# hliangzhao/torch-on-k8s

Hardware: AMD Instinct MI355X
Metric: tokens_per_s (higher is better)
Workload: dtype bf16; 1 GPU; model=llama3-8b, global_batch=8, seq_len=4096, parallelism=dp1, attn_impl=hip

## Files before the change

### torch_on_k8s_amd/models/llama.py

```python
from __future__ import annotations

import secrets
from dataclasses import dataclass, asdict

import torch
import torch.nn as nn
import torch.nn.functional as F

from torch_on_k8s_amd import ops


@dataclass
class LlamaConfig:
    name: str = "llama3-8b"
    vocab_size: int = 128256
    hidden_size: int = 4096
    intermediate_size: int = 14336
    num_layers: int = 32
    num_heads: int = 32
    num_kv_heads: int = 8
    head_dim: int = 128
    max_seq_len: int = 8192
    rope_theta: float = 500000.0
    rms_eps: float = 1e-5
    tie_embeddings: bool = False
    attn_impl: str = "hip"
    init_std: float = 0.02

    def to_dict(self):
        return asdict(self)


PRESETS = {
    "llama3-8b": LlamaConfig(),
    "llama-tiny": LlamaConfig(
        name="llama-tiny", vocab_size=512, hidden_size=256,
        intermediate_size=512, num_layers=2, num_heads=4, num_kv_heads=2,
        head_dim=64, max_seq_len=256, rope_theta=10000.0),
    "llama-1b": LlamaConfig(
        name="llama-1b", vocab_size=32000, hidden_size=2048,
        intermediate_size=5504, num_layers=16, num_heads=16, num_kv_heads=8,
        head_dim=128, max_seq_len=4096, rope_theta=500000.0),
}


def get_config(name: str, **overrides) -> LlamaConfig:
    cfg = PRESETS[name]
    if overrides:
        d = cfg.to_dict()
        d.update(overrides)
        cfg = LlamaConfig(**d)
    return cfg


class RMSNorm(nn.Module):
    def __init__(self, hidden: int, eps: float):
        super().__init__()
        self.weight = nn.Parameter(torch.ones(hidden))
        self.eps = eps

    def forward(self, x):
        return ops.rmsnorm(x, self.weight, self.eps)


def build_rope_table(cfg: LlamaConfig, seq_len: int, device) -> tuple[torch.Tensor, torch.Tensor]:
    half = cfg.head_dim // 2
    inv_freq = 1.0 / (cfg.rope_theta ** (torch.arange(0, half, dtype=torch.float64) / half))
    t = torch.arange(seq_len, dtype=torch.float64)
    ang = torch.outer(t, inv_freq)
    return (ang.cos().float().contiguous().to(device),
            ang.sin().float().contiguous().to(device))


class Attention(nn.Module):

    def __init__(self, cfg: LlamaConfig):
        super().__init__()
        self.cfg = cfg
        H, D = cfg.num_heads, cfg.head_dim
        Hkv = cfg.num_kv_heads
        self.qkv_proj = nn.Linear(cfg.hidden_size, (H + 2 * Hkv) * D,
                                  bias=False)
        self.o_proj = nn.Linear(H * D, cfg.hidden_size, bias=False)

    def project_qkv(self, x, cos, sin):
        cfg = self.cfg
        qkv = self.qkv_proj(x)
        return ops.qkv_rope(qkv, cos, sin, cfg.num_heads, cfg.num_kv_heads,
                            cfg.head_dim)

    def forward(self, x, cos, sin):
        B, S, _ = x.shape
        cfg = self.cfg
        q, k, v = self.project_qkv(x, cos, sin)
        if cfg.attn_impl == "sdpa" and x.is_cuda:
            rep = cfg.num_heads // cfg.num_kv_heads
            qt = q.transpose(1, 2)
            kt = k.transpose(1, 2).repeat_interleave(rep, dim=1)
            vt = v.transpose(1, 2).repeat_interleave(rep, dim=1)
            o = F.scaled_dot_product_attention(qt, kt, vt, is_causal=True)
            o = o.transpose(1, 2).contiguous()
        else:
            o = ops.attention(q, k, v, causal=True)
        return self.o_proj(o.reshape(B, S, cfg.num_heads * cfg.head_dim))


class MLP(nn.Module):

    def __init__(self, cfg: LlamaConfig):
        super().__init__()
        self.gate_up_proj = nn.Linear(cfg.hidden_size,
                                      2 * cfg.intermediate_size, bias=False)
        self.down_proj = nn.Linear(cfg.intermediate_size, cfg.hidden_size, bias=False)

    def forward(self, x):
        return self.down_proj(ops.swiglu(self.gate_up_proj(x)))


class Block(nn.Module):

    def __init__(self, cfg: LlamaConfig):
        super().__init__()
        self.input_norm = RMSNorm(cfg.hidden_size, cfg.rms_eps)
        self.attn = Attention(cfg)
        self.post_attn_norm = RMSNorm(cfg.hidden_size, cfg.rms_eps)
        self.mlp = MLP(cfg)

    def forward(self, x, res, cos, sin):
        h, xr = ops.rmsnorm_residual(x, res, self.input_norm.weight,
                                     self.input_norm.eps)
        a = self.attn(h, cos, sin)
        h2, xr2 = ops.rmsnorm_residual(a, xr, self.post_attn_norm.weight,
                                       self.post_attn_norm.eps)
        return self.mlp(h2), xr2


class LlamaModel(nn.Module):

    def __init__(self, cfg: LlamaConfig, activation_checkpointing: bool = False):
        super().__init__()
        self.cfg = cfg
        self.activation_checkpointing = activation_checkpointing
        self.embed_tokens = nn.Embedding(cfg.vocab_size, cfg.hidden_size)
        self.layers = nn.ModuleList(Block(cfg) for _ in range(cfg.num_layers))
        self.norm = RMSNorm(cfg.hidden_size, cfg.rms_eps)
        self.lm_head = nn.Linear(cfg.hidden_size, cfg.vocab_size, bias=False)
        if cfg.tie_embeddings:
            self.lm_head.weight = self.embed_tokens.weight
        self._rope_cache: tuple[int, torch.Tensor, torch.Tensor] | None = None
        self.reset_parameters()

    def reset_parameters(self):
        std = self.cfg.init_std
        for m in self.modules():
            if isinstance(m, nn.Linear):
                nn.init.normal_(m.weight, mean=0.0, std=std)
            elif isinstance(m, nn.Embedding):
                nn.init.normal_(m.weight, mean=0.0, std=std)
            elif isinstance(m, RMSNorm):
                nn.init.ones_(m.weight)
        scale = (2 * self.cfg.num_layers) ** -0.5
        for blk in self.layers:
            with torch.no_grad():
                blk.attn.o_proj.weight.mul_(scale)
                blk.mlp.down_proj.weight.mul_(scale)

    def _rope(self, S: int, device):
        if self._rope_cache is None or self._rope_cache[0] != S or \
                self._rope_cache[1].device != device:
            cos, sin = build_rope_table(self.cfg, S, device)
            self._rope_cache = (S, cos, sin)
        return self._rope_cache[1], self._rope_cache[2]

    def forward_hidden(self, input_ids: torch.Tensor) -> torch.Tensor:
        B, S = input_ids.shape
        cos, sin = self._rope(S, input_ids.device)
        x = self.embed_tokens(input_ids)
        res = None
        for blk in self.layers:
            if self.activation_checkpointing and self.training:
                x, res = torch.utils.checkpoint.checkpoint(
                    blk, x, res, cos, sin, use_reentrant=False)
            else:
                x, res = blk(x, res, cos, sin)
        y, _ = ops.rmsnorm_residual(x, res, self.norm.weight, self.norm.eps)
        return y

    def forward(self, input_ids: torch.Tensor,
                labels: torch.Tensor | None = None):
        x = self.forward_hidden(input_ids)
        logits = self.lm_head(x)
        if labels is None:
            return logits
        return ops.cross_entropy(logits, labels)

    @torch.no_grad()
    def generate(self, input_ids: torch.Tensor, max_new_tokens: int = 32,
                 temperature: float = 0.0,
                 use_graph: bool | None = None) -> torch.Tensor:
        cfg = self.cfg
        B, S0 = input_ids.shape
        dev = input_ids.device
        dtype = self.embed_tokens.weight.dtype
        Tmax = S0 + max_new_tokens
        Hkv, Hq, D = cfg.num_kv_heads, cfg.num_heads, cfg.head_dim
        kc = [torch.zeros(B, Tmax, Hkv, D, dtype=dtype, device=dev)
              for _ in self.layers]
        vc = [torch.zeros(B, Tmax, Hkv, D, dtype=dtype, device=dev)
              for _ in self.layers]
        cos, sin = build_rope_table(cfg, Tmax, dev)

        def run_block(blk, i, x, pos0, T):
            B_, s, _ = x.shape
            h = blk.input_norm(x)
            q, k, v = blk.attn.project_qkv(
                h, cos[pos0:pos0 + s].contiguous(),
                sin[pos0:pos0 + s].contiguous())
            kc[i][:, pos0:pos0 + s] = k
            vc[i][:, pos0:pos0 + s] = v
            if s > 1:
                o = ops.attention(q, k, v, causal=True)
            else:
                o = ops.attention_decode(q[:, 0], kc[i], vc[i], T)
                o = o.view(B_, 1, Hq, D)
            x = x + blk.attn.o_proj(o.reshape(B_, s, Hq * D))
            x = x + blk.mlp(blk.post_attn_norm(x))
            return x

        def next_token(logits):
            if temperature and temperature > 0:
                probs = torch.softmax(logits.float() / temperature, dim=-1)
                return torch.multinomial(probs, 1)
            return logits.argmax(-1, keepdim=True)

        x = self.embed_tokens(input_ids)
        for i, blk in enumerate(self.layers):
            x = run_block(blk, i, x, 0, S0)
        logits = self.lm_head(self.norm(x[:, -1:]))[:, -1]
        tokens = [next_token(logits)]

        if use_graph is None:
            use_graph = (dev.type == "cuda" and not temperature and
                         max_new_tokens >= 8)

        if not use_graph:
            for step in range(1, max_new_tokens):
                pos = S0 + step - 1
                x = self.embed_tokens(tokens[-1])
                for i, blk in enumerate(self.layers):
                    x = run_block(blk, i, x, pos, pos + 1)
                logits = self.lm_head(self.norm(x))[:, -1]
                tokens.append(next_token(logits))
            return torch.cat([input_ids] + tokens, dim=1)

        token_buf = tokens[0].clone()
        pos_long = torch.tensor([S0], dtype=torch.long, device=dev)
        t32 = torch.zeros((), dtype=torch.int32, device=dev)

        def decode_step():
            t32.copy_((pos_long[0] + 1).to(torch.int32))
            x = self.embed_tokens(token_buf)
            cs = torch.index_select(cos, 0, pos_long).contiguous()
            sn = torch.index_select(sin, 0, pos_long).contiguous()
            for i, blk in enumerate(self.layers):
                h = blk.input_norm(x)
                q, k, v = blk.attn.project_qkv(h, cs, sn)
                kc[i].index_copy_(1, pos_long, k)
                vc[i].index_copy_(1, pos_long, v)
                o = ops.attention_decode(q[:, 0], kc[i], vc[i], 0, T_dev=t32)
                x = x + blk.attn.o_proj(o.view(B, 1, Hq * D))
                x = x + blk.mlp(blk.post_attn_norm(x))
            logits = self.lm_head(self.norm(x))[:, -1]
            nxt = logits.argmax(-1, keepdim=True)
            token_buf.copy_(nxt)
# ... 164 lines not shown
```

### torch_on_k8s_amd/ops/__init__.py

```python
from __future__ import annotations

import torch

try:
    from . import _C
except ImportError:
    _C = None


def hip_ext_available() -> bool:
    return _C is not None


def _require_ext(op: str):
    if _C is None:
        raise RuntimeError(
            f"torch_on_k8s_amd HIP extension is required for {op} on GPU but "
            "is not built. Run: PYTORCH_ROCM_ARCH=gfx950 python setup.py "
            "build_ext --inplace"
        )
    return _C


def rmsnorm_ref(x: torch.Tensor, w: torch.Tensor, eps: float) -> torch.Tensor:
    xf = x.float()
    r = torch.rsqrt(xf.pow(2).mean(-1, keepdim=True) + eps)
    return (xf * r * w.float()).to(x.dtype)


class _RMSNormFn(torch.autograd.Function):
    @staticmethod
    def forward(ctx, x, w, eps):
        if x.is_cuda:
            y, invr = _require_ext("rmsnorm").rmsnorm_fwd(x, w, eps)
        else:
            xf = x.float()
            invr = torch.rsqrt(xf.pow(2).mean(-1) + eps).reshape(-1)
            y = (xf * invr.view(*x.shape[:-1], 1) * w.float()).to(x.dtype)
        ctx.save_for_backward(x, w, invr)
        return y

    @staticmethod
    def backward(ctx, dy):
        x, w, invr = ctx.saved_tensors
        dy = dy.contiguous()
        if x.is_cuda:
            dx, dw = _C.rmsnorm_bwd(x, w, dy, invr)
        else:
            xf, wf, dyf = x.float(), w.float(), dy.float()
            H = x.shape[-1]
            r = invr.view(*x.shape[:-1], 1)
            c = (dyf * wf * xf).sum(-1, keepdim=True)
            dx = (r * (wf * dyf - xf * (r * r / H) * c)).to(x.dtype)
            dw = (dyf * xf * r).reshape(-1, H).sum(0)
        return dx, dw.to(w.dtype), None


def rmsnorm(x: torch.Tensor, w: torch.Tensor, eps: float = 1e-5) -> torch.Tensor:
    return _RMSNormFn.apply(x.contiguous(), w, eps)


class _RMSNormResFn(torch.autograd.Function):

    @staticmethod
    def forward(ctx, x, res, w, eps):
        if x.is_cuda:
            y, xr, invr = _require_ext("rmsnorm_res").rmsnorm_res_fwd(
                x, res, w, eps)
        else:
            xr = x + res if res is not None else x
            xf = xr.float()
            invr = torch.rsqrt(xf.pow(2).mean(-1) + eps).reshape(-1)
            y = (xf * invr.view(*xr.shape[:-1], 1) * w.float()).to(x.dtype)
        ctx.save_for_backward(xr, w, invr)
        ctx.has_res = res is not None
        return y, xr

    @staticmethod
    def backward(ctx, dy, dxr):
        xr, w, invr = ctx.saved_tensors
        dy = dy.contiguous()
        if dxr is not None:
            dxr = dxr.contiguous()
# ... 392 lines not shown
        if logits.dtype != torch.bfloat16:
            raise TypeError(
                f"sample_tokens: GPU logits must be bfloat16, got "
                f"{logits.dtype}")
        return _require_ext("sample_tokens").sample_tokens(
            logits, temperature, top_k, top_p, seed, counter, u)
    B = logits.shape[0]
    out = torch.empty(B, dtype=torch.long)
    lf = logits.double()
    for b in range(B):
        ub = (float(u[b]) if u is not None
              else sample_uniform(int(seed[b]), int(counter[b])))
        out[b] = _sample_row_cpu(lf[b], float(temperature[b]), int(top_k[b]),
                                 float(top_p[b]), ub)
    return out


class _LayerNormFn(torch.autograd.Function):
    @staticmethod
    def forward(ctx, x, w, b, eps):
        if x.is_cuda:
            y, mu, rstd = _require_ext("layernorm").layernorm_fwd(x, w, b, eps)
        else:
            xf = x.float()
            mu = xf.mean(-1)
            var = xf.var(-1, unbiased=False)
            rstd = torch.rsqrt(var + eps)
            y = (((xf - mu.unsqueeze(-1)) * rstd.unsqueeze(-1)) * w.float() +
                 b.float()).to(x.dtype)
            mu, rstd = mu.reshape(-1), rstd.reshape(-1)
        ctx.save_for_backward(x, w, mu, rstd)
        return y

    @staticmethod
    def backward(ctx, dy):
        x, w, mu, rstd = ctx.saved_tensors
        dy = dy.contiguous()
        if x.is_cuda:
            dx, dw, db = _C.layernorm_bwd(x, w, dy, mu, rstd)
        else:
            H = x.shape[-1]
            xf, wf, dyf = x.float(), w.float(), dy.float()
            muv = mu.view(*x.shape[:-1], 1)
            rs = rstd.view(*x.shape[:-1], 1)
            xhat = (xf - muv) * rs
            dyw = dyf * wf
            a1 = dyw.mean(-1, keepdim=True)
            a2 = (dyw * xhat).mean(-1, keepdim=True)
            dx = (rs * (dyw - a1 - xhat * a2)).to(x.dtype)
            dw = (dyf * xhat).reshape(-1, H).sum(0)
            db = dyf.reshape(-1, H).sum(0)
        return dx, dw.to(w.dtype), db.to(w.dtype), None


def layernorm(x: torch.Tensor, w: torch.Tensor, b: torch.Tensor,
              eps: float = 1e-5) -> torch.Tensor:
    return _LayerNormFn.apply(x.contiguous(), w, b, eps)


class _FusedCEFn(torch.autograd.Function):
    @staticmethod
    def forward(ctx, logits, labels):
        loss, lse = _require_ext("cross_entropy").ce_fwd(logits, labels)
        ctx.save_for_backward(logits, labels, lse)
        return loss.mean()

    @staticmethod
    def backward(ctx, grad_out):
        logits, labels, lse = ctx.saved_tensors
        gscale = (grad_out.float() / logits.numel() * logits.size(-1)) \
            .reshape(())
        dlogits = _C.ce_bwd(logits, labels, lse, gscale.contiguous())
        return dlogits, None


def cross_entropy(logits: torch.Tensor, labels: torch.Tensor) -> torch.Tensor:
    if logits.is_cuda and logits.dtype == torch.bfloat16:
        return _FusedCEFn.apply(logits.contiguous().view(-1, logits.shape[-1]),
                                labels.reshape(-1).int())
    return torch.nn.functional.cross_entropy(
        logits.float().view(-1, logits.shape[-1]), labels.reshape(-1))


__all__ = [
    "rmsnorm", "rmsnorm_ref", "apply_rope", "rope_ref", "fused_adamw_",
    "attention", "attention_ref", "cross_entropy", "layernorm",
    "qkv_rope", "qkv_rope_ref", "swiglu", "swiglu_ref",
    "hip_ext_available",
    "grad_sumsq_blocks", "grad_sumsq_", "grad_norm_finalize_",
    "attention_decode_ragged", "qkv_rope_append_",
    "decode_ragged_splits", "decode_ragged_chunk",
    "sample_tokens", "sample_uniform", "philox4x32_10",
]
```

### torch_on_k8s_amd/ops/csrc/bindings.cpp

```cpp
#include <torch/extension.h>
#include <ATen/hip/impl/HIPStreamMasqueradingAsCUDA.h>
#include <hip/hip_runtime.h>

extern "C" {
hipError_t tok_rmsnorm_fwd(const void* x, const void* w, void* y, float* invr,
                           long nrows, int H, float eps, hipStream_t stream);
int tok_rmsnorm_dw_rsplit(long nrows, int H);
hipError_t tok_rmsnorm_bwd(const void* x, const void* w, const void* dy,
                           const float* invr, void* dx, float* dw_f32,
                           float* dw_ws, long nrows, int H,
                           hipStream_t stream);
hipError_t tok_rmsnorm_res_fwd(const void* x, const void* res, const void* w,
                               void* xr, void* y, float* invr, long nrows,
                               int H, float eps, hipStream_t stream);
hipError_t tok_rmsnorm_res_bwd(const void* xr, const void* w, const void* dy,
                               const void* dxr_in, const float* invr,
                               void* dx, float* dw_f32, float* dw_ws,
                               long nrows, int H, hipStream_t stream);
hipError_t tok_swiglu_fwd(const void* gu, void* out, long rows, int I,
                          hipStream_t stream);
hipError_t tok_swiglu_bwd(const void* dout, const void* gu, void* dgu,
                          long rows, int I, hipStream_t stream);
hipError_t tok_qkv_rope_fwd(const void* qkv, void* q, void* k, void* v,
                            const float* cos_tab, const float* sin_tab,
                            long tokens, int Hq, int Hkv, int D,
                            long S, hipStream_t stream);
hipError_t tok_qkv_rope_bwd(const void* dq, const void* dk, const void* dv,
                            void* dqkv, const float* cos_tab,
                            const float* sin_tab, long tokens, int Hq,
                            int Hkv, int D, long S,
                            hipStream_t stream);
hipError_t tok_rope(const void* x, void* y, const float* cos_tab,
                    const float* sin_tab, long rows_total, int heads, int D,
                    long S, float sign, hipStream_t stream);
hipError_t tok_adamw(void* p, const void* g, float* m, float* v, long n,
                     float lr, float beta1, float beta2, float eps, float wd,
                     int step, float gscale, const int* step_dev,
                     const float* lr_dev, const float* gscale_dev,
                     hipStream_t stream);
int tok_grad_sumsq_max_blocks();
int tok_grad_sumsq_blocks(long n);
hipError_t tok_grad_sumsq(const void* g, long n, float* partials, int nblocks,
                          hipStream_t stream);
hipError_t tok_grad_norm_finalize(const float* partials, long count,
                                  float inv_count, float clip, float* out,
                                  hipStream_t stream);
hipError_t tok_mfma_probe_16x16x32(const void* A, const void* B, float* D,
                                   hipStream_t stream);
hipError_t tok_mfma_probe_32x32x16(const void* A, const void* B, float* D,
                                   hipStream_t stream);
hipError_t tok_attn_fwd(const void* q, const void* k, const void* vt, void* o,
                        float* lse, int B, int S, int Hq, int Hkv, int D,
                        int S_pad, int causal, hipStream_t stream,
                        int variant);
hipError_t tok_attn_bwd(const void* q, const void* k, const void* v,
                        const void* o, const void* dout, const void* q_t,
                        const void* k_t, const void* dot_t, const float* lse,
                        float* dsum_ws, float* rc_ws, void* dq, void* dk,
                        void* dv, int B, int S, int Hq, int Hkv, int D,
                        int S_pad, int causal, hipStream_t stream, int split,
                        int dq_variant);
hipError_t tok_transpose_head(const void* in, void* out, int B, int S, int H,
                              int D, int S_pad, hipStream_t stream);
hipError_t tok_attn_decode(const void* q, const void* k, const void* v,
                           void* out, int B, int T, const int* T_dev,
                           int Tmax, int Hq, int Hkv, int D,
                           hipStream_t stream);
hipError_t tok_attn_decode_ragged(const void* q, const void* k, const void* v,
                                  const int* lens, void* out, float* ws,
                                  int B, int Tmax, int Hq, int Hkv, int D,
                                  int num_splits, int chunk,
                                  hipStream_t stream);
hipError_t tok_qkv_rope_append(const void* qkv, void* q, void* kcache,
                               void* vcache, const float* cos_tab,
                               const float* sin_tab, const int* pos, int B,
                               int Tmax, int Hq, int Hkv, int D,
                               hipStream_t stream);
int tok_sample_max_vocab();
hipError_t tok_sample_tokens(const void* logits, long row_stride,
                             const float* temperature, const int* top_k,
                             const float* top_p, const long long* seed,
                             const void* counter, int counter_is_64,
                             const float* u_opt, long long* out, int B, int V,
                             hipStream_t stream);
hipError_t tok_layernorm_fwd(const void* x, const void* w, const void* b,
                             void* y, float* mu, float* rstd, long nrows,
                             int H, float eps, hipStream_t stream);
hipError_t tok_layernorm_bwd(const void* x, const void* w, const void* dy,
                             const float* mu, const float* rstd, void* dx,
                             float* dw, float* db, long nrows, int H,
                             hipStream_t stream);
hipError_t tok_ce_fwd(const void* logits, const int* labels, float* loss,
                      float* lse, long rows, int V, hipStream_t stream);
hipError_t tok_ce_bwd(const void* logits, const int* labels, const float* lse,
                      const float* gscale, void* dlogits, long rows, int V,
                      hipStream_t stream);
}

namespace {

#define CHECK_BF16_CUDA(t)                                                    \
  TORCH_CHECK(t.is_cuda(), #t " must be on GPU");                             \
  TORCH_CHECK(t.scalar_type() == at::kBFloat16, #t " must be bf16");          \
  TORCH_CHECK(t.is_contiguous(), #t " must be contiguous")

#define TOK_HIP_OK(expr)                                                      \
  do {                                                                        \
    hipError_t _e = (expr);                                                   \
    TORCH_CHECK(_e == hipSuccess, "HIP kernel launch failed: ",               \
                hipGetErrorString(_e));                                       \
  } while (0)

hipStream_t current_stream() {
  return at::hip::getCurrentHIPStreamMasqueradingAsCUDA().stream();
}

std::vector<at::Tensor> rmsnorm_fwd(at::Tensor x, at::Tensor w, double eps) {
  CHECK_BF16_CUDA(x);
  CHECK_BF16_CUDA(w);
  const long H = x.size(-1);
  TORCH_CHECK(H % 8 == 0, "hidden dim must be a multiple of 8");
  TORCH_CHECK(w.numel() == H, "weight shape mismatch");
// ... 438 lines not shown

std::vector<at::Tensor> layernorm_fwd(at::Tensor x, at::Tensor w,
                                      at::Tensor b, double eps) {
  CHECK_BF16_CUDA(x);
  CHECK_BF16_CUDA(w);
  CHECK_BF16_CUDA(b);
  const long H = x.size(-1);
  TORCH_CHECK(H % 8 == 0, "hidden dim must be a multiple of 8");
  const long nrows = x.numel() / H;
  auto y = at::empty_like(x);
  auto mu = at::empty({nrows}, x.options().dtype(at::kFloat));
  auto rstd = at::empty({nrows}, x.options().dtype(at::kFloat));
  TOK_HIP_OK(tok_layernorm_fwd(x.data_ptr(), w.data_ptr(), b.data_ptr(),
                               y.data_ptr(), mu.data_ptr<float>(),
                               rstd.data_ptr<float>(), nrows, (int)H,
                               (float)eps, current_stream()));
  return {y, mu, rstd};
}

std::vector<at::Tensor> layernorm_bwd(at::Tensor x, at::Tensor w,
                                      at::Tensor dy, at::Tensor mu,
                                      at::Tensor rstd) {
  CHECK_BF16_CUDA(x);
  const long H = x.size(-1);
  const long nrows = x.numel() / H;
  auto dx = at::empty_like(x);
  auto dw = at::zeros({H}, x.options().dtype(at::kFloat));
  auto db = at::zeros({H}, x.options().dtype(at::kFloat));
  TOK_HIP_OK(tok_layernorm_bwd(x.data_ptr(), w.data_ptr(), dy.data_ptr(),
                               mu.data_ptr<float>(), rstd.data_ptr<float>(),
                               dx.data_ptr(), dw.data_ptr<float>(),
                               db.data_ptr<float>(), nrows, (int)H,
                               current_stream()));
  return {dx, dw, db};
}

std::vector<at::Tensor> ce_fwd(at::Tensor logits, at::Tensor labels) {
  CHECK_BF16_CUDA(logits);
  TORCH_CHECK(labels.scalar_type() == at::kInt && labels.is_cuda());
  const long V = logits.size(-1);
  TORCH_CHECK(V % 8 == 0, "vocab must be a multiple of 8");
  const long rows = logits.numel() / V;
  TORCH_CHECK(labels.numel() == rows);
  auto loss = at::empty({rows}, logits.options().dtype(at::kFloat));
  auto lse = at::empty({rows}, logits.options().dtype(at::kFloat));
  TOK_HIP_OK(tok_ce_fwd(logits.data_ptr(), labels.data_ptr<int>(),
                        loss.data_ptr<float>(), lse.data_ptr<float>(), rows,
                        (int)V, current_stream()));
  return {loss, lse};
}

at::Tensor ce_bwd(at::Tensor logits, at::Tensor labels, at::Tensor lse,
                  at::Tensor gscale) {
  CHECK_BF16_CUDA(logits);
  TORCH_CHECK(gscale.scalar_type() == at::kFloat && gscale.is_cuda());
  const long V = logits.size(-1);
  const long rows = logits.numel() / V;
  auto dlogits = at::empty_like(logits);
  TOK_HIP_OK(tok_ce_bwd(logits.data_ptr(), labels.data_ptr<int>(),
                        lse.data_ptr<float>(), gscale.data_ptr<float>(),
                        dlogits.data_ptr(), rows, (int)V, current_stream()));
  return dlogits;
}

at::Tensor mfma_probe(at::Tensor A, at::Tensor B) {
  CHECK_BF16_CUDA(A);
  CHECK_BF16_CUDA(B);
  if (A.size(0) == 16) {
    TORCH_CHECK(A.sizes() == at::IntArrayRef({16, 32}) &&
                B.sizes() == at::IntArrayRef({32, 16}));
    auto D = at::empty({16, 16}, A.options().dtype(at::kFloat));
    TOK_HIP_OK(tok_mfma_probe_16x16x32(A.data_ptr(), B.data_ptr(),
                                       D.data_ptr<float>(), current_stream()));
    return D;
  }
  TORCH_CHECK(A.sizes() == at::IntArrayRef({32, 16}) &&
              B.sizes() == at::IntArrayRef({16, 32}));
  auto D = at::empty({32, 32}, A.options().dtype(at::kFloat));
  TOK_HIP_OK(tok_mfma_probe_32x32x16(A.data_ptr(), B.data_ptr(),
                                     D.data_ptr<float>(), current_stream()));
  return D;
}

}

PYBIND11_MODULE(TORCH_EXTENSION_NAME, mod) {
  mod.def("mfma_probe", &mfma_probe, "MFMA 16x16x32 bf16 layout probe");
  mod.def("attn_fwd", &attn_fwd, "Flash attention forward (bf16, gfx950)",
          py::arg("q"), py::arg("k"), py::arg("v"), py::arg("causal"),
          py::arg("variant") = 0);
  mod.def("attn_bwd", &attn_bwd, "Flash attention backward (bf16, gfx950)",
          py::arg("q"), py::arg("k"), py::arg("v"), py::arg("o"),
          py::arg("lse"), py::arg("dout"), py::arg("causal"),
          py::arg("split") = false, py::arg("dq_variant") = 1);
  mod.def("ce_fwd", &ce_fwd, "Fused cross-entropy forward (bf16, gfx950)");
  mod.def("layernorm_fwd", &layernorm_fwd, "LayerNorm forward (bf16, gfx950)");
  mod.def("attn_decode", &attn_decode,
          "Single-token KV-cache attention decode (bf16, gfx950)",
          py::arg("q"), py::arg("kcache"), py::arg("vcache"), py::arg("T"),
          py::arg("T_dev") = py::none());
  mod.def("attn_decode_ragged", &attn_decode_ragged,
          "Per-sequence-length KV-cache attention decode (bf16, gfx950)",
          py::arg("q"), py::arg("kcache"), py::arg("vcache"), py::arg("lens"),
          py::arg("num_splits"), py::arg("chunk"));
  mod.def("qkv_rope_append_", &qkv_rope_append_,
          "One-token packed-QKV RoPE + KV-cache append (bf16, gfx950)");
  mod.def("sample_tokens", &sample_tokens,
          "Fused temperature / top-k / top-p sampler (bf16, gfx950)",
          py::arg("logits"), py::arg("temperature"), py::arg("top_k"),
          py::arg("top_p"), py::arg("seed"), py::arg("counter"),
          py::arg("u") = py::none());
  mod.def("layernorm_bwd", &layernorm_bwd, "LayerNorm backward (bf16, gfx950)");
  mod.def("ce_bwd", &ce_bwd, "Fused cross-entropy backward (bf16, gfx950)");
  mod.def("rmsnorm_fwd", &rmsnorm_fwd, "RMSNorm forward (bf16, gfx950)");
  mod.def("rmsnorm_bwd", &rmsnorm_bwd, "RMSNorm backward (bf16, gfx950)");
  mod.def("rmsnorm_res_fwd", &rmsnorm_res_fwd,
          "Fused residual-add + RMSNorm forward (bf16, gfx950)",
          py::arg("x"), py::arg("res"), py::arg("w"), py::arg("eps"));
  mod.def("rmsnorm_res_bwd", &rmsnorm_res_bwd,
          "Fused residual-add + RMSNorm backward (bf16, gfx950)",
          py::arg("xr"), py::arg("w"), py::arg("dy"), py::arg("dxr"),
          py::arg("invr"));
  mod.def("swiglu_fwd", &swiglu_fwd,
          "Fused SwiGLU over packed gate_up (bf16, gfx950)");
  mod.def("swiglu_bwd", &swiglu_bwd,
          "Fused SwiGLU backward (bf16, gfx950)");
  mod.def("qkv_rope_fwd", &qkv_rope_fwd,
          "Packed-QKV split + RoPE (bf16, gfx950)");
  mod.def("qkv_rope_bwd", &qkv_rope_bwd,
          "Packed-QKV gather + inverse RoPE (bf16, gfx950)");
  mod.def("rope", &rope, "Rotary embedding rotate-half (bf16, gfx950)");
  mod.def("adamw_", &adamw_, "Fused AdamW on a flat bucket (gfx950)",
          py::arg("p"), py::arg("g"), py::arg("m"), py::arg("v"),
          py::arg("lr"), py::arg("beta1"), py::arg("beta2"), py::arg("eps"),
          py::arg("wd"), py::arg("step"), py::arg("gscale"),
          py::arg("step_dev") = py::none(), py::arg("lr_dev") = py::none(),
          py::arg("gscale_dev") = py::none());
  mod.def("grad_sumsq_blocks", &grad_sumsq_blocks,
          "Partial slots grad_sumsq_ needs for a bucket of n elements");
  mod.def("grad_sumsq_max_blocks", &grad_sumsq_max_blocks,
          "Grid cap of grad_sumsq_");
  mod.def("grad_sumsq_", &grad_sumsq_,
          "Per-block sum of squares of a flat bf16 bucket (gfx950)");
  mod.def("grad_norm_finalize_", &grad_norm_finalize_,
          "Sum partials -> {norm, clip-folded grad scale} (gfx950)",
          py::arg("partials"), py::arg("out"), py::arg("inv_count"),
          py::arg("clip"));
}
```

### torch_on_k8s_amd/parallel/ddp.py

```python
from __future__ import annotations

from dataclasses import dataclass, field

import torch
import torch.distributed as dist

ALIGN = 64


@dataclass
class _Seg:
    param: torch.nn.Parameter
    offset: int
    numel: int


@dataclass
class Bucket:
    index: int
    decay: bool
    segs: list = field(default_factory=list)
    numel: int = 0
    flat_param: torch.Tensor | None = None
    flat_grad: torch.Tensor | None = None
    pending: int = 0
    work: object | None = None


def _pad(n: int) -> int:
    return (n + ALIGN - 1) // ALIGN * ALIGN


class FlatBucketModel:

    def __init__(self, module: torch.nn.Module, *, bucket_mb: int = 256,
                 process_group=None, overlap: bool = True,
                 no_decay_keywords=("norm", "bias")):
        self.module = module
        self.group = process_group
        self.overlap = overlap
        self.world_size = (dist.get_world_size(process_group)
                           if dist.is_initialized() else 1)

        seen = set()
        params: list[tuple[str, torch.nn.Parameter]] = []
        for name, p in module.named_parameters():
            if p.requires_grad and id(p) not in seen:
                seen.add(id(p))
                params.append((name, p))
        params.reverse()

        bucket_bytes = bucket_mb * (1 << 20)
        self.buckets: list[Bucket] = []
        open_buckets: dict[tuple, Bucket] = {}
        self._param_bucket: dict[int, Bucket] = {}
        for name, p in params:
            decay = not any(k in name.lower() for k in no_decay_keywords) \
                and p.dim() >= 2
            key = (p.dtype, decay)
            b = open_buckets.get(key)
            esize = p.element_size()
            if b is None or (b.numel + _pad(p.numel())) * esize > bucket_bytes:
                b = Bucket(index=len(self.buckets), decay=decay)
                b.dtype = p.dtype
                self.buckets.append(b)
                open_buckets[key] = b
            b.segs.append(_Seg(p, b.numel, p.numel()))
            b.numel += _pad(p.numel())
            self._param_bucket[id(p)] = b

        dev = params[0][1].device if params else torch.device("cpu")
        for b in self.buckets:
            dtype = b.segs[0].param.dtype
            b.flat_param = torch.zeros(b.numel, dtype=dtype, device=dev)
            b.flat_grad = torch.zeros(b.numel, dtype=dtype, device=dev)
            for s in b.segs:
                with torch.no_grad():
                    b.flat_param[s.offset:s.offset + s.numel].copy_(
                        s.param.data.reshape(-1))
                s.param.data = b.flat_param[s.offset:s.offset + s.numel] \
                    .view(s.param.shape)
                s.param.grad = b.flat_grad[s.offset:s.offset + s.numel] \
                    .view(s.param.shape)
            b.pending = len(b.segs)

        self.accumulate_only = False
        self._norm_ws = None
        self._norm_parts = None
        self.norm_out = None
        self._hooks = []
        if self.overlap and self.world_size > 1:
            self._register_hooks()

    def _register_hooks(self):
        for b in self.buckets:
            for s in b.segs:
                h = s.param.register_post_accumulate_grad_hook(
                    self._make_hook(b))
                self._hooks.append(h)

    def set_world(self, world_size: int):
        self.world_size = world_size
        if self.overlap and world_size > 1 and not self._hooks:
            self._register_hooks()

    def _make_hook(self, bucket: Bucket):
        def hook(_param):
            bucket.pending -= 1
            if bucket.pending == 0:
                bucket.pending = len(bucket.segs)
                if not self.accumulate_only and self.world_size > 1 and \
                        dist.is_initialized():
                    bucket.work = dist.all_reduce(
                        bucket.flat_grad, group=self.group, async_op=True)
        return hook

    def set_accumulate(self, accumulate: bool):
        self.accumulate_only = accumulate

    def zero_grads(self):
        for b in self.buckets:
            b.flat_grad.zero_()
            b.pending = len(b.segs)
            b.work = None

    def finish_grad_sync(self):
        if self.world_size <= 1:
            return
        for b in self.buckets:
            if b.work is not None:
                b.work.wait()
            else:
                dist.all_reduce(b.flat_grad, group=self.group)
            b.work = None

    def grad_norm(self) -> torch.Tensor:
        dev = self.buckets[0].flat_grad.device
        total = torch.zeros((), dtype=torch.float32, device=dev)
        for b in self.buckets:
            total += b.flat_grad.float().pow(2).sum()
        return total.sqrt() / self.world_size

    def alloc_norm_workspace(self):
        from torch_on_k8s_amd import ops
        if self.norm_out is not None:
            return
        dev = self.buckets[0].flat_grad.device
        slots = [ops.grad_sumsq_blocks(b.numel) for b in self.buckets]
        ws = torch.zeros(sum(slots), dtype=torch.float32, device=dev)
        self._norm_ws = ws
        self._norm_parts = list(ws.split(slots))
        self.norm_out = torch.zeros(2, dtype=torch.float32, device=dev)

    @torch.no_grad()
    def device_grad_norm(self, *, inv_count: float, clip: float):
        from torch_on_k8s_amd import ops
        if self.norm_out is None:
            if self.buckets[0].flat_grad.is_cuda and \
                    torch.cuda.is_current_stream_capturing():
                raise RuntimeError(
                    "alloc_norm_workspace() must run before graph capture")
            self.alloc_norm_workspace()
        for b, part in zip(self.buckets, self._norm_parts):
            ops.grad_sumsq_(b.flat_grad, part)
        ops.grad_norm_finalize_(self._norm_ws, self.norm_out,
                                inv_count=inv_count, clip=clip)
# ... 69 lines not shown
```

Measured before the change: 21000 tokens/s.

## Add custom HIP weight-gradient GEMM writing directly into flat gradient buckets

Replaces nn.Linear calls with a custom autograd linear whose backward computes the weight gradient in a new hand-written gfx950 MFMA kernel. The kernel uses 256x256 tiles, double-buffered global-to-LDS loads and XCD-aware grouped tile scheduling. When the parameter's grad is a view into the flat DDP bucket, it accumulates in place instead of allocating a temporary and adding. A per-shape dispatch table picks the kernel or falls back to BLAS, and an env var selects the mode. The risk is that the custom kernel could be slower than hipBLASLt for some shapes, and accumulation happens in bf16.

```diff
diff --git a/torch_on_k8s_amd/models/llama.py b/torch_on_k8s_amd/models/llama.py
--- a/torch_on_k8s_amd/models/llama.py
+++ b/torch_on_k8s_amd/models/llama.py
@@ -85,7 +85,7 @@
 
     def project_qkv(self, x, cos, sin):
         cfg = self.cfg
-        qkv = self.qkv_proj(x)
+        qkv = ops.linear(x, self.qkv_proj.weight)
         return ops.qkv_rope(qkv, cos, sin, cfg.num_heads, cfg.num_kv_heads,
                             cfg.head_dim)
 
@@ -102,7 +102,8 @@
             o = o.transpose(1, 2).contiguous()
         else:
             o = ops.attention(q, k, v, causal=True)
-        return self.o_proj(o.reshape(B, S, cfg.num_heads * cfg.head_dim))
+        return ops.linear(o.reshape(B, S, cfg.num_heads * cfg.head_dim),
+                          self.o_proj.weight)
 
 
 class MLP(nn.Module):
@@ -114,7 +115,8 @@
         self.down_proj = nn.Linear(cfg.intermediate_size, cfg.hidden_size, bias=False)
 
     def forward(self, x):
-        return self.down_proj(ops.swiglu(self.gate_up_proj(x)))
+        gu = ops.linear(x, self.gate_up_proj.weight)
+        return ops.linear(ops.swiglu(gu), self.down_proj.weight)
 
 
 class Block(nn.Module):
@@ -189,7 +191,7 @@
     def forward(self, input_ids: torch.Tensor,
                 labels: torch.Tensor | None = None):
         x = self.forward_hidden(input_ids)
-        logits = self.lm_head(x)
+        logits = ops.linear(x, self.lm_head.weight)
         if labels is None:
             return logits
         return ops.cross_entropy(logits, labels)
diff --git a/torch_on_k8s_amd/ops/__init__.py b/torch_on_k8s_amd/ops/__init__.py
--- a/torch_on_k8s_amd/ops/__init__.py
+++ b/torch_on_k8s_amd/ops/__init__.py
@@ -1,4 +1,6 @@
 from __future__ import annotations
+
+import os
 
 import torch
 
@@ -557,7 +559,115 @@
         logits.float().view(-1, logits.shape[-1]), labels.reshape(-1))
 
 
+_WGRAD_TILE = 256
+_WGRAD_TOKENS = 64
+_WGRAD_GROUP = 4
+
+_WGRAD_DISPATCH = {
+    (28672, 4096): 4,
+    (4096, 14336): 4,
+    (4096, 4096): 8,
+    (128256, 4096): 4,
+    (6144, 4096): "blas",
+}
+
+
+def wgrad_impl() -> str:
+    impl = os.environ.get("TOK_WGRAD_IMPL", "hip").lower()
+    if impl not in ("hip", "hip_all", "blas"):
+        raise ValueError(
+            f"TOK_WGRAD_IMPL must be hip, hip_all or blas, got {impl!r}")
+    return impl
+
+
+def wgrad_band(N: int, K: int) -> int | None:
+    impl = wgrad_impl()
+    band = _WGRAD_DISPATCH.get((N, K))
+    if impl == "hip_all":
+        return band if isinstance(band, int) else _WGRAD_GROUP
+    if impl == "hip" and isinstance(band, int):
+        return band
+    return None
+
+
+def wgrad_fast_path(dy: torch.Tensor, x: torch.Tensor,
+                    out: torch.Tensor) -> bool:
+    if not (dy.is_cuda and x.is_cuda and out.is_cuda):
+        return False
+    if dy.dim() != 2 or x.dim() != 2 or out.dim() != 2:
+        return False
+    M, N = dy.shape
+    K = x.shape[1]
+    return (all(t.dtype == torch.bfloat16 and t.is_contiguous() and
+                t.data_ptr() % 16 == 0 for t in (dy, x, out))
+            and M >= _WGRAD_TOKENS and M % _WGRAD_TOKENS == 0
+            and N >= _WGRAD_TILE and N % _WGRAD_TILE == 0
+            and K >= _WGRAD_TILE and K % _WGRAD_TILE == 0)
+
+
+@torch.no_grad()
+def wgrad_gemm_(dy: torch.Tensor, x: torch.Tensor, out: torch.Tensor,
+                accumulate: bool, *, group: int | None = None) -> torch.Tensor:
+    if x.shape[0] != dy.shape[0] or out.shape != (dy.shape[1], x.shape[1]):
+        raise ValueError(
+            f"wgrad_gemm_: dy {tuple(dy.shape)}, x {tuple(x.shape)}, "
+            f"out {tuple(out.shape)} do not fit out[N,K] = dy[M,N]^T x[M,K]")
+    if group is None:
+        group = wgrad_band(*out.shape)
+    if group is not None and wgrad_fast_path(dy, x, out):
+        _require_ext("wgrad_gemm_").wgrad_gemm_(
+            dy, x, out, bool(accumulate), int(group))
+        return out
+    g = torch.mm(dy.t(), x)
+    if accumulate:
+        out.add_(g)
+    else:
+        out.copy_(g)
+    return out
+
+
+def _grad_in_place(weight: torch.Tensor) -> bool:
+    return (getattr(weight, "_tok_flat_grad", False)
+            and weight.grad is not None
+            and not getattr(weight, "_post_accumulate_grad_hooks", None)
+            and not getattr(weight, "_backward_hooks", None))
+
+
+class _LinearFn(torch.autograd.Function):
+
+    @staticmethod
+    def forward(ctx, x, weight):
+        ctx.save_for_backward(x, weight)
+        ctx.param = weight
+        return torch.nn.functional.linear(x, weight)
+
+    @staticmethod
+    def backward(ctx, dy):
+        x, weight = ctx.saved_tensors
+        param = ctx.param
+        N, K = weight.shape
+        dx = dw = None
+        dy2 = dy.reshape(-1, N)
+        if ctx.needs_input_grad[0]:
+            dx = dy2.mm(weight).view(x.shape)
+        if ctx.needs_input_grad[1]:
+            dy2 = dy2.contiguous()
+            x2 = x.reshape(-1, K).contiguous()
+            if _grad_in_place(param) and param.grad.dtype == dy2.dtype:
+                wgrad_gemm_(dy2, x2, param.grad, True)
+            else:
+                dw = wgrad_gemm_(dy2, x2, torch.empty_like(weight), False)
+        return dx, dw
+
+
+def linear(x: torch.Tensor, weight: torch.Tensor) -> torch.Tensor:
+    if wgrad_impl() == "blas":
+        return torch.nn.functional.linear(x, weight)
+    return _LinearFn.apply(x, weight)
+
+
 __all__ = [
+    "linear", "wgrad_gemm_", "wgrad_fast_path", "wgrad_impl", "wgrad_band",
     "rmsnorm", "rmsnorm_ref", "apply_rope", "rope_ref", "fused_adamw_",
     "attention", "attention_ref", "cross_entropy", "layernorm",
     "qkv_rope", "qkv_rope_ref", "swiglu", "swiglu_ref",
diff --git a/torch_on_k8s_amd/ops/csrc/bindings.cpp b/torch_on_k8s_amd/ops/csrc/bindings.cpp
--- a/torch_on_k8s_amd/ops/csrc/bindings.cpp
+++ b/torch_on_k8s_amd/ops/csrc/bindings.cpp
@@ -38,6 +38,9 @@
                      int step, float gscale, const int* step_dev,
                      const float* lr_dev, const float* gscale_dev,
                      hipStream_t stream);
+hipError_t tok_wgrad_gemm(const void* dy, const void* x, void* c, long M,
+                          long N, long K, int accumulate, int group,
+                          hipStream_t stream);
 int tok_grad_sumsq_max_blocks();
 int tok_grad_sumsq_blocks(long n);
 hipError_t tok_grad_sumsq(const void* g, long n, float* partials, int nblocks,
@@ -642,6 +645,28 @@
   return D;
 }
 
+}
+
+void wgrad_gemm_(at::Tensor dy, at::Tensor x, at::Tensor out, bool accumulate,
+                 int64_t group) {
+  CHECK_BF16_CUDA(dy);
+  CHECK_BF16_CUDA(x);
+  CHECK_BF16_CUDA(out);
+  TORCH_CHECK(dy.dim() == 2 && x.dim() == 2 && out.dim() == 2,
+              "wgrad_gemm_: dy, x and out must be 2-D");
+  const long M = dy.size(0), N = dy.size(1), K = x.size(1);
+  TORCH_CHECK(x.size(0) == M && out.size(0) == N && out.size(1) == K,
+              "wgrad_gemm_: need dy [M,N], x [M,K], out [N,K]");
+  TORCH_CHECK(M >= 64 && M % 64 == 0 && N >= 256 && N % 256 == 0 &&
+                  K >= 256 && K % 256 == 0,
+              "wgrad_gemm_: needs M % 64 == 0 and N, K multiples of 256");
+  TORCH_CHECK(((uintptr_t)dy.data_ptr() | (uintptr_t)x.data_ptr() |
+               (uintptr_t)out.data_ptr()) % 16 == 0,
+              "wgrad_gemm_: pointers must be 16-byte aligned");
+  TORCH_CHECK(group >= 1, "wgrad_gemm_: group must be >= 1");
+  TOK_HIP_OK(tok_wgrad_gemm(dy.data_ptr(), x.data_ptr(), out.data_ptr(), M, N,
+                            K, accumulate ? 1 : 0, (int)group,
+                            current_stream()));
 }
 
 PYBIND11_MODULE(TORCH_EXTENSION_NAME, mod) {
@@ -706,4 +731,8 @@
           "Sum partials -> {norm, clip-folded grad scale} (gfx950)",
           py::arg("partials"), py::arg("out"), py::arg("inv_count"),
           py::arg("clip"));
-}
+  mod.def("wgrad_gemm_", &wgrad_gemm_,
+          "out[N,K] (+)= dy[M,N]^T x[M,K], bf16, fp32 accumulate (gfx950)",
+          py::arg("dy"), py::arg("x"), py::arg("out"), py::arg("accumulate"),
+          py::arg("group"));
+}
diff --git a/torch_on_k8s_amd/ops/csrc/wgrad_gemm.hip b/torch_on_k8s_amd/ops/csrc/wgrad_gemm.hip
--- /dev/null
+++ b/torch_on_k8s_amd/ops/csrc/wgrad_gemm.hip
@@ -0,0 +1,286 @@
+#include "common.h"
+
+namespace {
+
+using bf16x8v = __attribute__((ext_vector_type(8))) __bf16;
+using bf16x4v = __attribute__((ext_vector_type(4))) __bf16;
+using i16x4v = __attribute__((ext_vector_type(4))) short;
+using f32x4 = __attribute__((ext_vector_type(4))) float;
+
+constexpr int WG_TILE = 256;
+constexpr int WG_BK = 64;
+constexpr int WG_NTH = 512;
+constexpr int UNIT_BYTES = 64 * 256;
+constexpr int BUF_STRIDE = UNIT_BYTES;
+constexpr int U_ALO = 0 * 2 * UNIT_BYTES;
+constexpr int U_AHI = 1 * 2 * UNIT_BYTES;
+constexpr int U_BLO = 2 * 2 * UNIT_BYTES;
+constexpr int U_BHI = 3 * 2 * UNIT_BYTES;
+constexpr int EPI_LD = 68;
+constexpr int WG_LDS_BYTES = 8 * 64 * EPI_LD * 4;
+static_assert(WG_LDS_BYTES >= 8 * UNIT_BYTES, "epilogue image covers staging");
+
+typedef __attribute__((address_space(3))) i16x4v* lds_tr_ptr;
+
+DEVINL i16x4v tr_read(const char* p) {
+  return __builtin_amdgcn_ds_read_tr16_b64_v4i16((lds_tr_ptr)p);
+}
+
+DEVINL bf16x8v frag(i16x4v lo, i16x4v hi) {
+  union { i16x4v s[2]; bf16x8v f; } c;
+  c.s[0] = lo;
+  c.s[1] = hi;
+  return c.f;
+}
+
+DEVINL void glds16(uint32_t voff, const void* sbase, uint32_t lds_dst) {
+  uint32_t keep;
+  asm volatile(
+      "s_mov_b32 %0, m0\n\ts_mov_b32 m0, %3\n\ts_nop 0\n\t"
+      "global_load_lds_dwordx4 %1, %2\n\ts_mov_b32 m0, %0"
+      : "=&s"(keep)
+      : "v"(voff), "s"(sbase), "s"(lds_dst)
+      : "memory");
+}
+
+DEVINL void wg_barrier() {
+  __builtin_amdgcn_sched_barrier(0);
+  asm volatile("s_barrier" ::: "memory");
+  __builtin_amdgcn_sched_barrier(0);
+}
+
+struct WgCtx {
+  const char* lds;
+  uint32_t lds_u32;
+  uint32_t ra[2][4];
+  uint32_t rb[2][2];
+  uint32_t vdy[2], vx[2];
+  const char* dy0;
+  const char* x0;
+  long dy_step, x_step;
+  int last;
+};
+
+template <int UNIT, int BUF>
+DEVINL void stage_unit(const WgCtx& c, const char* src, const uint32_t (&v)[2]) {
+  const uint32_t dst = c.lds_u32 + UNIT + BUF * BUF_STRIDE;
+  glds16(v[0], src, dst);
+  glds16(v[1], src, dst + 8192);
+}
+
+template <int UNIT, int BUF>
+DEVINL void read_a(const WgCtx& c, bf16x8v (&a)[4][2]) {
+#pragma unroll
+  for (int mi = 0; mi < 4; ++mi)
+#pragma unroll
+    for (int s = 0; s < 2; ++s) {
+      const int o = UNIT + BUF * BUF_STRIDE + s * 8192;
+      a[mi][s] = frag(tr_read(c.lds + c.ra[0][mi] + o),
+                      tr_read(c.lds + c.ra[1][mi] + o));
+    }
+}
+
+template <int UNIT, int BUF>
+DEVINL void read_b(const WgCtx& c, bf16x8v (&b)[2][2]) {
+#pragma unroll
+  for (int ni = 0; ni < 2; ++ni)
+#pragma unroll
+    for (int s = 0; s < 2; ++s) {
+      const int o = UNIT + BUF * BUF_STRIDE + s * 8192;
+      b[ni][s] = frag(tr_read(c.lds + c.rb[0][ni] + o),
+                      tr_read(c.lds + c.rb[1][ni] + o));
+    }
+}
+
+template <int MH, int NH>
+DEVINL void mma_quadrant(f32x4 (&acc)[8][4], const bf16x8v (&a)[4][2],
+                         const bf16x8v (&b)[2][2]) {
+  wg_barrier();
+  asm volatile("s_waitcnt lgkmcnt(0)" ::: "memory");
+  __builtin_amdgcn_sched_barrier(0);
+  __builtin_amdgcn_s_setprio(1);
+#pragma unroll
+  for (int s = 0; s < 2; ++s)
+#pragma unroll
+    for (int mi = 0; mi < 4; ++mi)
+#pragma unroll
+      for (int ni = 0; ni < 2; ++ni)
+        acc[MH * 4 + mi][NH * 2 + ni] = __builtin_amdgcn_mfma_f32_16x16x32_bf16(
+            a[mi][s], b[ni][s], acc[MH * 4 + mi][NH * 2 + ni], 0, 0, 0);
+  __builtin_amdgcn_s_setprio(0);
+  wg_barrier();
+}
+
+template <int BUF>
+DEVINL void wgrad_tile(const WgCtx& c, int t, f32x4 (&acc)[8][4]) {
+  bf16x8v a[4][2], b0[2][2], b1[2][2];
+  const long t1 = min(t + 1, c.last), t2 = min(t + 2, c.last);
+  const char* dy1 = c.dy0 + t1 * c.dy_step;
+  const char* dy2 = c.dy0 + t2 * c.dy_step;
+  const char* x2 = c.x0 + t2 * c.x_step;
+
+  read_a<U_ALO, BUF>(c, a);
+  read_b<U_BLO, BUF>(c, b0);
+  stage_unit<U_AHI, BUF ^ 1>(c, dy1 + 256, c.vdy);
+  mma_quadrant<0, 0>(acc, a, b0);
+
+  read_b<U_BHI, BUF>(c, b1);
+  stage_unit<U_ALO, BUF>(c, dy2, c.vdy);
+  mma_quadrant<0, 1>(acc, a, b1);
+
+  read_a<U_AHI, BUF>(c, a);
+  stage_unit<U_BLO, BUF>(c, x2, c.vx);
+  mma_quadrant<1, 1>(acc, a, b1);
+
+  stage_unit<U_BHI, BUF>(c, x2 + 256, c.vx);
+  asm volatile("s_waitcnt vmcnt(6)" ::: "memory");
+  mma_quadrant<1, 0>(acc, a, b0);
+}
+
+__global__ __launch_bounds__(WG_NTH, 2) void wgrad_gemm_kernel(
+    const bf16_t* __restrict__ dy, const bf16_t* __restrict__ x,
+    bf16_t* __restrict__ C, int T, int N, int K, int accumulate, int group) {
+  __shared__ __attribute__((aligned(1024))) char smem[WG_LDS_BYTES];
+
+  const int tid = threadIdx.x;
+  const int lane = tid & 63;
+  const int wid = __builtin_amdgcn_readfirstlane(tid >> 6);
+  const int wr = wid >> 2, wc = wid & 3;
+
+  const unsigned TN = N / WG_TILE, TK = K / WG_TILE;
+  unsigned w;
+  {
+    const unsigned nwg = gridDim.x, l = blockIdx.x;
+    const unsigned q = nwg >> 3, r = nwg & 7, xcd = l & 7;
+    w = (xcd < r ? xcd * (q + 1) : r * (q + 1) + (xcd - r) * q) + (l >> 3);
+  }
+  unsigned tn, tk;
+  {
+    const unsigned per = (unsigned)group * TK;
+    const unsigned first = (w / per) * group;
+    const unsigned gsz = min(TN - first, (unsigned)group);
+    const unsigned rem = w % per;
+    tn = first + rem % gsz;
+    tk = rem / gsz;
+  }
+  const long n0 = (long)tn * WG_TILE, k0 = (long)tk * WG_TILE;
+
+  WgCtx c;
+  c.lds = smem;
+  c.lds_u32 = (uint32_t)(uintptr_t)(__attribute__((address_space(3))) char*)
+                  smem + wid * 1024;
+  c.lds_u32 = __builtin_amdgcn_readfirstlane(c.lds_u32);
+  {
+    const int g = lane >> 4, q = (lane >> 2) & 3, p = lane & 3;
+#pragma unroll
+    for (int u = 0; u < 2; ++u) {
+      const int row = 8 * g + 4 * u + q;
+      const int f = (q << 2) | ((2 * g + u) & 3);
+      const uint32_t base = 256 * row + 8 * (p & 1);
+      const uint32_t xo = 16 * ((p >> 1) ^ f);
+#pragma unroll
+      for (int mi = 0; mi < 4; ++mi)
+        c.ra[u][mi] = base + (xo ^ (32 * (4 * wr + mi)));
+#pragma unroll
+      for (int ni = 0; ni < 2; ++ni)
+        c.rb[u][ni] = base + (xo ^ (32 * (2 * wc + ni)));
+    }
+  }
+  {
+    const int row = tid >> 4, slot = tid & 15;
+    const int f = ((row & 3) << 2) | ((row >> 2) & 3);
+    const uint32_t ch = slot ^ f;
+    c.vdy[0] = (uint32_t)row * N * 2 + ch * 16;
+    c.vdy[1] = c.vdy[0] + 32u * N * 2;
+    c.vx[0] = (uint32_t)row * K * 2 + ch * 16;
+    c.vx[1] = c.vx[0] + 32u * K * 2;
+  }
+  c.dy0 = (const char*)(dy + n0);
+  c.x0 = (const char*)(x + k0);
+  c.dy_step = (long)WG_BK * N * 2;
+  c.x_step = (long)WG_BK * K * 2;
+  c.last = T - 1;
+
+  f32x4 acc[8][4];
+#pragma unroll
+  for (int i = 0; i < 8; ++i)
+#pragma unroll
+    for (int j = 0; j < 4; ++j) acc[i][j] = f32x4{0.f, 0.f, 0.f, 0.f};
+
+  {
+    const long t1 = min(1, c.last);
+    const char* dy1 = c.dy0 + t1 * c.dy_step;
+    const char* x1 = c.x0 + t1 * c.x_step;
+    stage_unit<U_ALO, 0>(c, c.dy0, c.vdy);
+    stage_unit<U_BLO, 0>(c, c.x0, c.vx);
+    stage_unit<U_BHI, 0>(c, c.x0 + 256, c.vx);
+    stage_unit<U_AHI, 0>(c, c.dy0 + 256, c.vdy);
+    stage_unit<U_ALO, 1>(c, dy1, c.vdy);
+    stage_unit<U_BLO, 1>(c, x1, c.vx);
+    stage_unit<U_BHI, 1>(c, x1 + 256, c.vx);
+    asm volatile("s_waitcnt vmcnt(6)" ::: "memory");
+    wg_barrier();
+  }
+
+  int t = 0;
+  for (; t + 1 < T; t += 2) {
+    wgrad_tile<0>(c, t, acc);
+    wgrad_tile<1>(c, t + 1, acc);
+  }
+  if (t < T) wgrad_tile<0>(c, t, acc);
+
+  asm volatile("s_waitcnt vmcnt(0)" ::: "memory");
+  __syncthreads();
+  float* ep = (float*)smem + wid * 64 * EPI_LD;
+  const int fr = lane & 15, fq = lane >> 4;
+  const int orow = lane >> 3, ocol = (lane & 7) * 8;
+  const long ccol = k0 + (ocol >> 5) * 128 + wc * 32 + (ocol & 31);
+#pragma unroll
+  for (int h = 0; h < 2; ++h) {
+#pragma unroll
+    for (int mi = 0; mi < 4; ++mi)
+#pragma unroll
+      for (int ni = 0; ni < 4; ++ni)
+#pragma unroll
+        for (int j = 0; j < 4; ++j)
+          ep[(mi * 16 + fq * 4 + j) * EPI_LD + ni * 16 + fr] =
+              acc[h * 4 + mi][ni][j];
+#pragma unroll
+    for (int it = 0; it < 8; ++it) {
+      const int row = it * 8 + orow;
+      const float* src = ep + row * EPI_LD + ocol;
+      const f32x4 v0 = *(const f32x4*)src;
+      const f32x4 v1 = *(const f32x4*)(src + 4);
+      float v[8] = {v0[0], v0[1], v0[2], v0[3], v1[0], v1[1], v1[2], v1[3]};
+      bf16_t* dst = C + (n0 + h * 128 + wr * 64 + row) * (long)K + ccol;
+      if (accumulate) {
+        const bf16x8 old = *(const bf16x8*)dst;
+#pragma unroll
+        for (int e = 0; e < 8; ++e) v[e] += bfbits2f(old.h[e]);
+      }
+      bf16x8 o;
+#pragma unroll
+      for (int e = 0; e < 8; ++e) o.h[e] = f2bfbits(v[e]);
+      *(bf16x8*)dst = o;
+    }
+  }
+}
+
+}
+
+extern "C" hipError_t tok_wgrad_gemm(const void* dy, const void* x, void* c,
+                                     long M, long N, long K, int accumulate,
+                                     int group, hipStream_t stream) {
+  if (M < WG_BK || M % WG_BK || N < WG_TILE || N % WG_TILE || K < WG_TILE ||
+      K % WG_TILE || group < 1)
+    return hipErrorInvalidValue;
+  if (64 * (N > K ? N : K) * 2 >= (1L << 31) || M / WG_BK >= (1L << 30))
+    return hipErrorInvalidValue;
+  const long tiles = (N / WG_TILE) * (K / WG_TILE);
+  if (tiles >= (1L << 30)) return hipErrorInvalidValue;
+  if (group > N / WG_TILE) group = (int)(N / WG_TILE);
+  wgrad_gemm_kernel<<<dim3((unsigned)tiles), WG_NTH, 0, stream>>>(
+      (const bf16_t*)dy, (const bf16_t*)x, (bf16_t*)c, (int)(M / WG_BK),
+      (int)N, (int)K, accumulate, group);
+  return hipGetLastError();
+}
diff --git a/torch_on_k8s_amd/parallel/ddp.py b/torch_on_k8s_amd/parallel/ddp.py
--- a/torch_on_k8s_amd/parallel/ddp.py
+++ b/torch_on_k8s_amd/parallel/ddp.py
@@ -82,6 +82,7 @@
                     .view(s.param.shape)
                 s.param.grad = b.flat_grad[s.offset:s.offset + s.numel] \
                     .view(s.param.shape)
+                s.param._tok_flat_grad = True
             b.pending = len(b.segs)
 
         self.accumulate_only = False
```

Result: faster. 21650 tokens/s (median of 6 runs) (+3.1%).
